# facebookresearch/seamless_communication

Measured on AMD Instinct MI355X. Metric: S2ST utterances/sec (and real-time factor), seamlessM4T_v2_large, 10 s audio, higher is better.
Workload: dtype f32 activations x f16 weights, f32 accumulate

## Files before the change

### include/seamless_hip_internal.h

```cpp
#ifndef SEAMLESS_HIP_INTERNAL_H_
#define SEAMLESS_HIP_INTERNAL_H_

#include "seamless_hip.h"

#ifdef __cplusplus
extern "C" {
#endif

int sc_decoder_step_family(sc_model* m, int rows, int caller);

int sc_op_knob(const char* name, int dflt);

int sc_op_force_general_gemm(int on);
int32_t sc_op_voc_pack_plan(const int32_t* h_need, int32_t n, int64_t budget_rows, int32_t* h_group_first, int32_t cap);
int32_t sc_op_voc_tile_first(const int32_t* h_off, int32_t n, int32_t mul, int32_t tile_rows, int32_t* h_first);
int32_t sc_op_last_vocoder_packed_groups(sc_model* m);
int sc_op_single_plane(int on);
int sc_op_layernorm(const float* d_x, const float* d_gamma, const float* d_beta, float* d_y, int32_t rows, int32_t C,
                    int32_t act);
int sc_op_linear(const float* d_x, const void* d_w_f16, const float* d_bias, const float* d_res, float* d_y,
                 int32_t M, int32_t N, int32_t K, int32_t act, float alpha, int32_t split, int32_t force_gemv);
int sc_op_skinny_linear(const float* d_x, const void* d_w_f16, const float* d_bias, const float* d_res, float* d_y,
                        int32_t M, int32_t N, int32_t K, int32_t act, float alpha);
int sc_op_skinny_res_ln(const float* d_in, const void* d_w_f16, const float* d_bias, float* d_x_inout,
// ... 42 lines not shown
int sc_op_xattn_rows(const float* d_q, int64_t ldq, const float* d_k, int64_t ldk, int32_t n, int32_t s1, int32_t s_enc, int32_t heads,
                     const int32_t* h_enc_lens, const int32_t* h_tok_lens, float* d_xattn);
int32_t sc_op_xattn_rows_tile(int32_t which);
int sc_op_conv1d_presplit(const float* d_x, const void* d_w_f16_packed, const float* d_bias, const float* d_res, float* d_y,
                          void* d_yh_f16, void* d_yl_f16, int32_t nb, int32_t t, int32_t cin, int32_t cout, int32_t k, int32_t pad,
                          int32_t dil, const unsigned char* d_row_valid, int32_t act);
int sc_op_resblock_pair_ps(const float* d_x, const void* d_w1_packed, const float* d_b1, const void* d_w2_packed, const float* d_b2,
                           float* d_out, int32_t nb, int32_t T, int32_t C, int32_t k, int32_t dil);
int sc_op_resblock_pair(const float* d_x, const void* d_w1_packed, const float* d_b1, const void* d_w2_packed,
                        const float* d_b2, float* d_out, int32_t nb, int32_t T, int32_t C, int32_t k, int32_t dil,
                        float slope, const float* d_avg_a, const float* d_avg_b);
int sc_op_mrf_fused(const float* d_x, const void* const* d_w1_packed, const float* const* d_b1, const void* const* d_w2_packed,
                    const float* const* d_b2, float* d_out, int32_t nb, int32_t T, int32_t C, const int32_t* k, const int32_t* dil,
                    float slope);
int sc_op_attention(const float* d_q, const float* d_k, const float* d_v, float* d_out, int32_t nb, int32_t heads,
                    int32_t sq, int32_t skv, int64_t ldq, int64_t ldk, int64_t ldv, int64_t ldo,
                    const int32_t* d_kv_lens, int32_t causal, const float* d_rel_k, int32_t rel_left,
                    int32_t rel_right);
int sc_op_attention_ex(const float* d_q, const float* d_k, const float* d_v, float* d_out, int32_t nb, int32_t heads,
                       int32_t sq, int32_t skv, int64_t ldq, int64_t ldk, int64_t ldv, int64_t ldo,
                       const int32_t* d_kv_lens, int32_t causal, const float* d_rel_k, int32_t rel_left,
                       int32_t rel_right, const int32_t* d_row_off, const float* d_rp_table, int64_t rp_ld,
                       const float* d_q_bias_u, const float* d_q_bias_v, void* d_out_hi, void* d_out_lo, int64_t ldoh);
int sc_op_glu_dwconv(const float* d_x, const float* d_w, float* d_y, int32_t nb, int32_t T, int32_t C, int32_t k,
                     const int32_t* d_lens);
int sc_op_glu_dwconv_ln(const float* d_x, const float* d_w, const float* d_gamma, const float* d_beta, int32_t act, void* d_yh_f16,
                        void* d_yl_f16, int32_t nb, int32_t T, int32_t C, int32_t k, const int32_t* d_lens, int32_t fused);
int sc_op_layernorm2(const float* d_x, const float* d_ga, const float* d_ba, const float* d_gb, const float* d_bb, float* d_y,
                     void* d_yh_f16, void* d_yl_f16, int32_t rows, int32_t C, int32_t fused);
int sc_op_argmax(const float* d_logits, int32_t rows, int32_t V, int32_t* d_idx, float* d_lprob);

int sc_op_beam_candidates(float* d_logits, int64_t ld, int32_t n_utt, int32_t beams, int32_t V, const float* d_cum, int32_t first_step,
                          int32_t no_eos, int32_t force_eos, int32_t pad_idx, int32_t eos_idx, int32_t unk_idx, float unk_penalty, int32_t K,
                          float* d_cand_val, int32_t* d_cand_idx, const int32_t* d_seqs, int32_t seq_ld, int32_t S, int32_t G,
                          const int32_t* d_rows, const int32_t* d_slots, int32_t chunked);
int sc_op_beam_candidates_banned(float* d_logits, int64_t ld, int32_t n_utt, int32_t beams, int32_t V, const float* d_cum,
                                 int32_t first_step, int32_t no_eos, int32_t force_eos, int32_t pad_idx, int32_t eos_idx, int32_t unk_idx,
                                 float unk_penalty, int32_t K, float* d_cand_val, int32_t* d_cand_idx, const int32_t* d_seqs,
                                 int32_t seq_ld, int32_t S, int32_t G, const int32_t* d_rows, const int32_t* d_slots, int32_t chunked,
                                 const int32_t* d_banned_tokens, const int32_t* d_banned_offsets, int32_t n_banned);
int sc_op_sample_rows(float* d_logits, int64_t ld, int32_t rows, int32_t V, const uint64_t* d_stream, const int32_t* d_gen,
                      const int32_t* d_position, float temperature, int32_t top_k, float top_p, uint64_t seed, int32_t no_eos, int32_t force_eos,
                      int32_t pad_idx, int32_t eos_idx, int32_t unk_idx, float unk_penalty, const int32_t* d_seqs, int32_t seq_ld, int32_t S,
                      int32_t G, const int32_t* d_banned_tokens, const int32_t* d_banned_offsets, int32_t n_banned, int32_t* d_tok,
                      float* d_lprob, int32_t* d_kept, uint64_t* d_z_kept);
int sc_op_beam_select(const float* d_cand_val, const int32_t* d_cand_idx, const int32_t* d_seqs_cur, int32_t* d_seqs_new, float* d_fin_score,
// ... 104 lines not shown
```

### seamless_communication_amd/_lib.py

```python
from __future__ import annotations

import ctypes as C
from pathlib import Path
from typing import Optional

import os

_VARIANT = os.environ.get("SC_LIB_VARIANT", "")
LIB_PATH = Path(__file__).resolve().parent / (f"libseamless_hip.{_VARIANT}.so" if _VARIANT else "libseamless_hip.so")

SC_ABI_VERSION = 10
SC_MAX_UPSAMPLES = 8
SC_MAX_RESBLOCK_KERNELS = 4
SC_MAX_RESBLOCK_DILATIONS = 4
SC_F16, SC_F32, SC_I32 = 0, 1, 2


class SeamlessHipError(RuntimeError):
    pass


class sc_tensor_desc(C.Structure):
    _fields_ = [
        ("name", C.c_char_p),
# ... 257 lines not shown
    "sc_op_glu_dwconv_ln": (C.c_int, [_P, _P, _P, _P, _i, _P, _P, _i, _i, _i, _i, _P, _i]),
    "sc_op_layernorm2": (C.c_int, [_P, _P, _P, _P, _P, _P, _P, _P, _i, _i, _i]),
    "sc_op_dstep3_gemv": (C.c_int, [_i, _P, _P, _P, _P, _P, _P, _P, _P, _i, _i, _i, _i, _i, _i]),
    "sc_op_dstep3_argmax": (C.c_int, [_P, _P, _i, _i, _i, _i, _i, _i, _i, _i, _i, C.c_float, _P, _P]),
    "sc_op_chain_bench": (C.c_int, [_i, _i, _i, _i, _P]),
    "sc_op_dstep_attention": (C.c_int, [_P, _i, _P, _P, _P, _i, _i, _P, _i, _i, _i, _P]),
    "sc_op_conv1d": (C.c_int, [_P, _P, _P, _P, _P, _i, _i, _i, _i, _i, _i, _i, _i, _P, _i, _i]),
    "sc_op_pack_conv_weight": (C.c_int, [_P, _P, _i, _i, _i]),
    "sc_op_conv_transpose1d": (C.c_int, [_P, _P, _P, _P, _P, _i, _i, _i, _i, _i, _i, _i, _i]),
    "sc_op_linear_presplit": (C.c_int, [_P, _P, _P, _P, _P, _P, _P, _i, _i, _i, _i, C.c_float]),
    "sc_op_linear_presplit_argmax": (C.c_int, [_P, _P, _P, _P, _i, _i, _i]),
    "sc_op_linear_presplit_score": (C.c_int, [_P, _P, _P, _P, _P, _P, _P, _P, _i, _i, _i]),
    "sc_op_linear_presplit_score_grouped": (C.c_int, [_P, _P, _P, _P, _P, _P, _P, _P, _i, _i, _i, _i]),
    "sc_op_score_candidates": (C.c_int, [_P, _P, _P, _P, _i, _P, _P, _i, _i, _i]),
    "sc_op_score_record_cols": (_i, [_i]),
    "sc_op_score_group_rows": (_i, [_i]),
    "sc_op_conv1d_presplit": (C.c_int, [_P, _P, _P, _P, _P, _P, _P, _i, _i, _i, _i, _i, _i, _i, _P, _i]),
    "sc_op_mrf_fused": (C.c_int, [_P, _P, _P, _P, _P, _P, _i, _i, _i, _P, _P, C.c_float]),
    "sc_op_resblock_pair": (C.c_int, [_P, _P, _P, _P, _P, _P, _i, _i, _i, _i, _i, C.c_float, _P, _P]),
    "sc_op_attention": (C.c_int, [_P, _P, _P, _P, _i, _i, _i, _i, C.c_int64, C.c_int64, C.c_int64, C.c_int64, _P, _i,
                                  _P, _i, _i]),
    "sc_op_attention_ex": (C.c_int, [_P, _P, _P, _P, _i, _i, _i, _i, C.c_int64, C.c_int64, C.c_int64, C.c_int64, _P, _i,
                                     _P, _i, _i, _P, _P, C.c_int64, _P, _P, _P, _P, C.c_int64]),
    "sc_op_glu_dwconv": (C.c_int, [_P, _P, _P, _i, _i, _i, _i, _P]),
    "sc_op_argmax": (C.c_int, [_P, _i, _i, _P, _P]),
    "sc_op_beam_candidates": (C.c_int, [_P, C.c_int64, _i, _i, _i, _P, _i, _i, _i, _i, _i, _i, C.c_float, _i, _P, _P, _P, _i, _i, _i,
                                        _P, _P, _i]),
    "sc_op_beam_candidates_banned": (C.c_int, [_P, C.c_int64, _i, _i, _i, _P, _i, _i, _i, _i, _i, _i, C.c_float, _i, _P, _P, _P, _i, _i,
                                               _i, _P, _P, _i, _P, _P, _i]),
    "sc_op_sample_rows": (C.c_int, [_P, C.c_int64, _i, _i, _P, _P, _P, C.c_float, _i, C.c_float, C.c_uint64, _i, _i, _i, _i, _i, C.c_float,
                                    _P, _i, _i, _i, _P, _P, _i, _P, _P, _P, _P]),
    "sc_op_beam_select": (C.c_int, [_P, _P, _P, _P, _P, _P, _P, _P, _P, _P, _P, _P, _P, _P, _i, _P, _P, _i, _i, _i, _i, _i, _i, _i, _i,
                                    _i, C.c_float]),
    "sc_op_beam_compact": (C.c_int, [_P, _P, _P, _P, _P, _P, _P, _P, _P, _i, _i, _i, _i, _i, _i]),
    "sc_op_gather_cache": (C.c_int, [_P, _P, _P, _i, _i, _i, _i, _i, C.c_int64]),
    "sc_op_row_token_lprob": (C.c_int, [_P, C.c_int64, _i, _i, _i, _i, _P]),
    "sc_op_dstep_attention_ex": (C.c_int, [_P, _i, _P, _P, _P, _i, _i, _i, _P, _i, _i, _i, _P, _P, _P, _P, _i, _P, _P]),
    "sc_op_engine_step_close": (C.c_int, [_P, _P, _i, _i, _i, _i, _i, _i, _i, C.c_float, _P, _P, _i, _i, _P, _P, _P, _P, _P, _P, _P, _P]),
    "sc_op_engine_admit": (C.c_int, [_P, _i, _i, _i, _i, _P, _P, _P, _P, _P, _P, _P, _P, _P]),
    "sc_op_engine_set_slots": (C.c_int, [_P, _i, _i, _i, _P, _P, _P, _P]),
    "sc_op_engine_retire": (C.c_int, [_P, _P, _P, _i, _i, _i, _i, _P, _P, _P, _P, _P]),
    "sc_op_dstep3_embed_ex": (C.c_int, [_P, _P, C.c_float, _P, _i, _P, _P, _i, _i, _i, _i, _i, _P]),
    "sc_op_dstep3_reduce_capture_ex": (C.c_int, [_P, _i, _P, _P, _P, _P, _P, _P, C.c_int64, _i, _i, _P, _P, _i, _i, _i]),
    "sc_op_step_update": (C.c_int, [_P, _P, _i, _P, _P, _P, _P, _i, _i, _i, _i, _P]),
    "sc_op_row_swap": (C.c_int, [_P, _P, _P, _i, _i, _P, _P, _i, _i, _i, _i, _i, _P, _P, _P, _P, _P, _P, _P, _P]),
}
# ... 92 lines not shown
```

### seamless_communication_amd/csrc/api.hip

```cpp
#include <atomic>
#include <cstring>
#include <map>
#include <mutex>
#include <set>

#include "engine.h"
#include "handle.h"

using namespace sc;

struct sc_model {
    Model m;
    sc_config& cfg = m.cfg;
};

struct sc_engine {
    std::unique_ptr<Engine> e;
    int device = 0;
    const void* weights = nullptr;
    std::set<sc_model*> attached;
};

static std::mutex g_attach_mu;
static std::map<Engine*, sc_engine*> g_engine_owner;
// ... 1453 lines not shown
    SC_CHECK(d_x && d_w1_packed && d_b1 && d_w2_packed && d_b2 && d_out && k && dil, "sc_op_mrf_fused: null argument");
    MrfArgs a;
    a.x = d_x;
    a.out = d_out;
    a.nb = nb;
    a.T = T;
    a.C = C;
    a.slope = slope;
    for (int j = 0; j < 3; ++j) a.k[j] = k[j];
    for (int q = 0; q < 9; ++q) {
        a.dil[q] = dil[q];
        a.w1[q] = static_cast<const __half*>(d_w1_packed[q]);
        a.w2[q] = static_cast<const __half*>(d_w2_packed[q]);
        a.ldw1[q] = a.ldw2[q] = align_up((int64_t)C * k[q / 3], 32);
        a.b1[q] = d_b1[q];
        a.b2[q] = d_b2[q];
    }
    a.single = g_op_single.load();
    launch_mrf_fused(a, g_op_stream);
    SC_HIP(hipStreamSynchronize(g_op_stream));
    SC_API_END
}

int sc_op_attention(const float* d_q, const float* d_k, const float* d_v, float* d_out, int32_t nb, int32_t heads,
                    int32_t sq, int32_t skv, int64_t ldq, int64_t ldk, int64_t ldv, int64_t ldo, const int32_t* d_kv_lens,
                    int32_t causal, const float* d_rel_k, int32_t rel_left, int32_t rel_right) {
    SC_API_BEGIN
    AttnArgs a;
    a.q = d_q;
    a.k = d_k;
    a.v = d_v;
    a.out = d_out;
    a.ldq = ldq;
    a.ldk = ldk;
    a.ldv = ldv;
    a.ldo = ldo;
    a.nb = nb;
    a.heads = heads;
    a.Sq = sq;
    a.Skv = skv;
    a.kv_lens = d_kv_lens;
    a.causal = causal;
    a.rel_k = d_rel_k;
    a.rel_left = rel_left;
    a.rel_right = rel_right;
    launch_attention(a, g_op_stream);
    SC_HIP(hipStreamSynchronize(g_op_stream));
    SC_API_END
}

int sc_op_attention_ex(const float* d_q, const float* d_k, const float* d_v, float* d_out, int32_t nb, int32_t heads,
                       int32_t sq, int32_t skv, int64_t ldq, int64_t ldk, int64_t ldv, int64_t ldo, const int32_t* d_kv_lens,
                       int32_t causal, const float* d_rel_k, int32_t rel_left, int32_t rel_right, const int32_t* d_row_off,
                       const float* d_rp_table, int64_t rp_ld, const float* d_q_bias_u, const float* d_q_bias_v, void* d_out_hi,
                       void* d_out_lo, int64_t ldoh) {
    SC_API_BEGIN
    AttnArgs a;
    a.q = d_q;
    a.k = d_k;
    a.v = d_v;
    a.out = d_out;
    a.ldq = ldq;
    a.ldk = ldk;
    a.ldv = ldv;
    a.ldo = ldo;
    a.nb = nb;
    a.heads = heads;
    a.Sq = sq;
    a.Skv = skv;
    a.kv_lens = d_kv_lens;
    a.causal = causal;
    a.rel_k = d_rel_k;
    a.rel_left = rel_left;
    a.rel_right = rel_right;
    a.row_off = d_row_off;
    a.rp_table = d_rp_table;
    a.rp_ld = rp_ld;
    a.q_bias_u = d_q_bias_u;
    a.q_bias_v = d_q_bias_v;
    a.out_hi = static_cast<__half*>(d_out_hi);
// ... 495 lines not shown
```

### seamless_communication_amd/csrc/k_attn.hip

```cpp
#include <cstdlib>

#include "device_util.h"

namespace sc {

static constexpr int HD = 64;

static constexpr int MQ = 128;
static constexpr int MKV = 32;
static constexpr int KS = 68;
static constexpr int KH_LD = 72;
static constexpr int VT_LD = 40;

template <int MODE>
__global__ __launch_bounds__(256) void attn_mfma16_kernel(AttnArgs p) {
    constexpr bool SHAW = MODE == 1;
    constexpr bool RELPOS = MODE == 2;
    extern __shared__ __attribute__((aligned(16))) float smem[];
    _Float16* sKh = reinterpret_cast<_Float16*>(smem);
    _Float16* sKl = sKh + MKV * KH_LD;
    _Float16* sVh = sKl + MKV * KH_LD;
    _Float16* sVl = sVh + HD * VT_LD;
    float* sQR = smem + 4 * 32 * KS;
    float* sT = smem + 4 * 32 * KS;
    float* sR = smem;

    const int tid = threadIdx.x, lane = tid & 63, wave = tid >> 6;
    const int ql = lane & 31, hh = lane >> 5;
    int qb = blockIdx.x, h = blockIdx.y, n = blockIdx.z;
    {
        const int gx = gridDim.x, bh_all = gridDim.y * gridDim.z;
        if ((bh_all & 7) == 0) {
            const int L = blockIdx.x + gx * (blockIdx.y + gridDim.y * blockIdx.z);
            const int bh = (L / (8 * gx)) * 8 + (L & 7);
            qb = (L >> 3) % gx;
            h = bh % gridDim.y;
            n = bh / gridDim.y;
        }
    }
    const int q0 = qb * MQ + wave * 32;
    const int qi = q0 + ql;
    const int kv_len = p.kv_lens ? min(p.kv_lens[n], p.Skv) : p.Skv;
    const int shift = p.Skv - p.Sq;
    const int qabs = qi + shift;
    const int npos = p.rel_left + 1 + p.rel_right;
    const int sq_n = p.row_off ? kv_len : p.Sq;
    const int64_t qbase = p.row_off ? (int64_t)p.row_off[n] : (int64_t)n * p.Sq;
    const int64_t kvbase = p.row_off ? (int64_t)p.row_off[n] : (int64_t)n * p.Skv;
    if (p.row_off && qb * MQ >= kv_len) return;
    const bool qok = qi < sq_n;
    const float* qrow = p.q + (qbase + (qok ? qi : 0)) * p.ldq + h * HD;

    if (SHAW) {
        float qreg[32];
#pragma unroll
        for (int g = 0; g < 8; ++g) {
            f32x4_t v = {0.f, 0.f, 0.f, 0.f};
            if (qok) v = *reinterpret_cast<const f32x4_t*>(qrow + 8 * g + 4 * hh);
            qreg[4 * g + 0] = v[0];
            qreg[4 * g + 1] = v[1];
            qreg[4 * g + 2] = v[2];
            qreg[4 * g + 3] = v[3];
        }
        for (int idx = tid; idx < npos * (HD / 4); idx += 256) {
            const int r = idx >> 4, c4 = idx & 15;
            *reinterpret_cast<f32x4_t*>(&sR[r * KS + c4 * 4]) = *reinterpret_cast<const f32x4_t*>(p.rel_k + r * HD + c4 * 4);
        }
        __syncthreads();
#pragma unroll 1
        for (int f = 0; f < 3; ++f) {
            if (f * 32 >= npos) break;
            float16_t qr;
#pragma unroll
            for (int r = 0; r < 16; ++r) qr[r] = 0.f;
#pragma unroll
            for (int g = 0; g < 8; ++g) {
                const f32x4_t r4 = *reinterpret_cast<const f32x4_t*>(&sR[(f * 32 + ql) * KS + 8 * g + 4 * hh]);
                qr = __builtin_amdgcn_mfma_f32_32x32x2f32(r4[0], qreg[4 * g + 0], qr, 0, 0, 0);
                qr = __builtin_amdgcn_mfma_f32_32x32x2f32(r4[1], qreg[4 * g + 1], qr, 0, 0, 0);
                qr = __builtin_amdgcn_mfma_f32_32x32x2f32(r4[2], qreg[4 * g + 2], qr, 0, 0, 0);
                qr = __builtin_amdgcn_mfma_f32_32x32x2f32(r4[3], qreg[4 * g + 3], qr, 0, 0, 0);
            }
#pragma unroll
            for (int r = 0; r < 16; ++r) {
                const int e = f * 32 + (r & 3) + 8 * (r >> 2) + 4 * hh;
                if (e < npos) sQR[(wave * 32 + ql) * npos + e] = qr[r];
            }
        }
    }

    half8_t qh[4], qlo[4], qvh[RELPOS ? 4 : 1], qvl[RELPOS ? 4 : 1];
#pragma unroll
    for (int c = 0; c < 4; ++c) {
        float x[8];
#pragma unroll
        for (int e = 0; e < 8; ++e) x[e] = 0.f;
        if (qok) {
            const f32x4_t v0 = *reinterpret_cast<const f32x4_t*>(qrow + 16 * c + 8 * hh);
            const f32x4_t v1 = *reinterpret_cast<const f32x4_t*>(qrow + 16 * c + 8 * hh + 4);
#pragma unroll
            for (int e = 0; e < 4; ++e) {
                x[e] = v0[e];
                x[4 + e] = v1[e];
            }
        }
        if (RELPOS) {
            float xu[8], xv[8];
#pragma unroll
            for (int e = 0; e < 8; ++e) {
                xu[e] = x[e] + p.q_bias_u[h * HD + 16 * c + 8 * hh + e];
                xv[e] = x[e] + p.q_bias_v[h * HD + 16 * c + 8 * hh + e];
            }
            split8(xu, qh[c], qlo[c]);
            split8(xv, qvh[c], qvl[c]);
        } else {
            split8(x, qh[c], qlo[c]);
        }
    }

    float16_t o0, o1;
#pragma unroll
    for (int r = 0; r < 16; ++r) {
        o0[r] = 0.f;
        o1[r] = 0.f;
    }
    float m_i = -1e30f, l_i = 0.f;

    int k_end = kv_len;
    if (p.causal) k_end = min(k_end, qb * MQ + MQ - 1 + shift + 1);

    const int sr0 = tid >> 4, sc4 = tid & 15;
    f32x4_t kf[2], vf[2];
    auto fetch = [&](int k0) {
#pragma unroll
        for (int u = 0; u < 2; ++u) {
            const int r = sr0 + 16 * u;
            kf[u] = f32x4_t{0.f, 0.f, 0.f, 0.f};
            vf[u] = kf[u];
            if (k0 + r < kv_len) {
                const int64_t row = kvbase + k0 + r;
                kf[u] = *reinterpret_cast<const f32x4_t*>(p.k + row * p.ldk + h * HD + sc4 * 4);
                vf[u] = *reinterpret_cast<const f32x4_t*>(p.v + row * p.ldv + h * HD + sc4 * 4);
            }
        }
    };
    if (k_end > 0) fetch(0);

    for (int k0 = 0; k0 < k_end; k0 += MKV) {
        __syncthreads();
#pragma unroll
        for (int u = 0; u < 2; ++u) {
            const int r = sr0 + 16 * u;
            half4_t khi, klo, vhi, vlo;
#pragma unroll
            for (int e = 0; e < 4; ++e) {
                const _Float16 a = (_Float16)kf[u][e];
                khi[e] = a;
                klo[e] = (_Float16)(kf[u][e] - (float)a);
                const _Float16 b = (_Float16)vf[u][e];
                vhi[e] = b;
                vlo[e] = (_Float16)(vf[u][e] - (float)b);
            }
            *reinterpret_cast<half4_t*>(&sKh[r * KH_LD + 4 * sc4]) = khi;
            *reinterpret_cast<half4_t*>(&sKl[r * KH_LD + 4 * sc4]) = klo;
            const int w = r & 15;
            const int pos = (r & 16) + 8 * ((w >> 2) & 1) + (w & 3) + 4 * (w >> 3);
#pragma unroll
            for (int e = 0; e < 4; ++e) {
                sVh[(4 * sc4 + e) * VT_LD + pos] = vhi[e];
                sVl[(4 * sc4 + e) * VT_LD + pos] = vlo[e];
            }
        }
        if (k0 + MKV < k_end) fetch(k0 + MKV);
        __syncthreads();

        float qr[16];
        if (SHAW) {
            const float* qrow_t = sQR + (wave * 32 + ql) * npos;
            const int rel_max = k0 + (MKV - 1) - (q0 + shift);
            const int rel_min = k0 - (q0 + 31 + shift);
            if (rel_max <= -p.rel_left) {
                const float v = qrow_t[0];
#pragma unroll
                for (int r = 0; r < 16; ++r) qr[r] = v;
            } else if (rel_min >= p.rel_right) {
                const float v = qrow_t[npos - 1];
#pragma unroll
                for (int r = 0; r < 16; ++r) qr[r] = v;
            } else {
#pragma unroll
                for (int r = 0; r < 16; ++r) {
                    const int kj = k0 + (r & 3) + 8 * (r >> 2) + 4 * hh;
                    const int rel = max(-p.rel_left, min(p.rel_right, kj - qabs)) + p.rel_left;
                    qr[r] = qrow_t[rel];
                }
            }
        }
        if (RELPOS) {
            const int t0w = (p.Skv - 1) - (q0 + shift) + k0 - 31;
            const int t_max = 2 * p.Skv - 2;
            float* tw = sT + wave * (64 * 32);
#pragma unroll
            for (int blk = 0; blk < 2; ++blk) {
                const int trow = min(max(t0w + blk * 32 + ql, 0), t_max);
                const float* rrow = p.rp_table + (int64_t)trow * p.rp_ld + h * HD + 8 * hh;
                f32x4_t ra[4][2];
#pragma unroll
                for (int c = 0; c < 4; ++c) {
                    ra[c][0] = *reinterpret_cast<const f32x4_t*>(rrow + 16 * c);
                    ra[c][1] = *reinterpret_cast<const f32x4_t*>(rrow + 16 * c + 4);
                }
                float16_t tt;
#pragma unroll
                for (int r = 0; r < 16; ++r) tt[r] = 0.f;
#pragma unroll
                for (int c = 0; c < 4; ++c) {
                    float x[8];
#pragma unroll
                    for (int e = 0; e < 4; ++e) {
                        x[e] = ra[c][0][e];
                        x[4 + e] = ra[c][1][e];
                    }
                    half8_t rh, rl;
                    split8(x, rh, rl);
                    tt = __builtin_amdgcn_mfma_f32_32x32x16_f16(rh, qvh[c], tt, 0, 0, 0);
                    tt = __builtin_amdgcn_mfma_f32_32x32x16_f16(rh, qvl[c], tt, 0, 0, 0);
                    tt = __builtin_amdgcn_mfma_f32_32x32x16_f16(rl, qvh[c], tt, 0, 0, 0);
                }
#pragma unroll
                for (int r = 0; r < 16; ++r) tw[(blk * 32 + (r & 3) + 8 * (r >> 2) + 4 * hh) * 32 + ql] = tt[r];
            }
#pragma unroll
            for (int r = 0; r < 16; ++r) {
                const int jl = (r & 3) + 8 * (r >> 2) + 4 * hh;
                qr[r] = tw[(jl - ql + 31) * 32 + ql];
            }
        }
        float16_t st;
#pragma unroll
        for (int r = 0; r < 16; ++r) st[r] = 0.f;
#pragma unroll
        for (int c = 0; c < 4; ++c) {
            const half8_t kh = *reinterpret_cast<const half8_t*>(&sKh[ql * KH_LD + 16 * c + 8 * hh]);
            const half8_t kl = *reinterpret_cast<const half8_t*>(&sKl[ql * KH_LD + 16 * c + 8 * hh]);
            st = __builtin_amdgcn_mfma_f32_32x32x16_f16(kh, qh[c], st, 0, 0, 0);
            st = __builtin_amdgcn_mfma_f32_32x32x16_f16(kh, qlo[c], st, 0, 0, 0);
            st = __builtin_amdgcn_mfma_f32_32x32x16_f16(kl, qh[c], st, 0, 0, 0);
        }
        float mx = -INFINITY;
#pragma unroll
        for (int r = 0; r < 16; ++r) {
            const int kj = k0 + (r & 3) + 8 * (r >> 2) + 4 * hh;
            float sc = st[r];
            if (SHAW || RELPOS) sc += qr[r];
            const bool ok = (kj < kv_len) && (!p.causal || kj <= qabs);
            sc = sc * 0.125f + (ok ? 0.f : -INFINITY);
            st[r] = sc;
            mx = fmaxf(mx, sc);
        }
        mx = fmaxf(mx, __shfl_xor(mx, 32));
        const float m_new = fmaxf(m_i, mx);
        constexpr float LOG2E = 1.44269504088896340736f;
        const float alpha = __builtin_amdgcn_exp2f((m_i - m_new) * LOG2E);
        float rs = 0.f;
#pragma unroll
        for (int r = 0; r < 16; ++r) {
            const float pv = __builtin_amdgcn_exp2f((st[r] - m_new) * LOG2E);
            st[r] = pv;
            rs += pv;
        }
        rs += __shfl_xor(rs, 32);
        l_i = l_i * alpha + rs;
        m_i = m_new;
        if (__builtin_amdgcn_ballot_w64(alpha != 1.f) != 0) {
#pragma unroll
            for (int r = 0; r < 16; ++r) {
                o0[r] *= alpha;
                o1[r] *= alpha;
            }
        }
#pragma unroll
        for (int c = 0; c < 2; ++c) {
            float x[8];
#pragma unroll
            for (int e = 0; e < 8; ++e) x[e] = st[8 * c + e];
            half8_t ph, pl;
            split8(x, ph, pl);
            const half8_t v0h = *reinterpret_cast<const half8_t*>(&sVh[ql * VT_LD + 16 * c + 8 * hh]);
            const half8_t v0l = *reinterpret_cast<const half8_t*>(&sVl[ql * VT_LD + 16 * c + 8 * hh]);
            const half8_t v1h = *reinterpret_cast<const half8_t*>(&sVh[(32 + ql) * VT_LD + 16 * c + 8 * hh]);
            const half8_t v1l = *reinterpret_cast<const half8_t*>(&sVl[(32 + ql) * VT_LD + 16 * c + 8 * hh]);
            o0 = __builtin_amdgcn_mfma_f32_32x32x16_f16(v0h, ph, o0, 0, 0, 0);
            o1 = __builtin_amdgcn_mfma_f32_32x32x16_f16(v1h, ph, o1, 0, 0, 0);
            o0 = __builtin_amdgcn_mfma_f32_32x32x16_f16(v0h, pl, o0, 0, 0, 0);
            o1 = __builtin_amdgcn_mfma_f32_32x32x16_f16(v1h, pl, o1, 0, 0, 0);
            o0 = __builtin_amdgcn_mfma_f32_32x32x16_f16(v0l, ph, o0, 0, 0, 0);
            o1 = __builtin_amdgcn_mfma_f32_32x32x16_f16(v1l, ph, o1, 0, 0, 0);
        }
    }

    __syncthreads();
    float* ot = smem + wave * (32 * KS);
    const float inv = l_i > 0.f ? 1.0f / l_i : 0.f;
#pragma unroll
    for (int r = 0; r < 16; ++r) {
        const int d = (r & 3) + 8 * (r >> 2) + 4 * hh;
        ot[ql * KS + d] = o0[r] * inv;
        ot[ql * KS + 32 + d] = o1[r] * inv;
    }
#pragma unroll
    for (int it = 0; it < 8; ++it) {
        const int row = it * 4 + (lane >> 4);
        const int c0 = (lane & 15) * 4;
        const int qq = q0 + row;
        const f32x4_t of = *reinterpret_cast<const f32x4_t*>(&ot[row * KS + c0]);
        if (qq >= sq_n) continue;
        if (p.out_hi) {
            const half4_t hi = __builtin_convertvector(of, half4_t);
            const f32x4_t back = __builtin_convertvector(hi, f32x4_t);
            const int64_t off = (qbase + qq) * p.ldoh + h * HD + c0;
            *reinterpret_cast<half4_t*>(p.out_hi + off) = hi;
            *reinterpret_cast<half4_t*>(p.out_lo + off) = __builtin_convertvector(of - back, half4_t);
        } else {
            *reinterpret_cast<f32x4_t*>(p.out + (qbase + qq) * p.ldo + h * HD + c0) = of;
        }
    }
}

static bool g_attn_attr_set = false;

void launch_attention(const AttnArgs& a, hipStream_t s) {
    if (a.head_dim == 80 || a.head_dim == 128) {
        launch_attention_hd(a, s);
        return;
    }
    SC_CHECK(a.head_dim == HD, "attention: head_dim=%d (64, 80 and 128 exist)", a.head_dim);
    SC_CHECK(a.nb > 0 && a.heads > 0 && a.Sq > 0 && a.Skv > 0, "attention: empty problem");
    SC_CHECK(a.out || (a.out_hi && a.out_lo && a.ldoh % 4 == 0), "attention: no output");
    SC_CHECK(a.ldq % 4 == 0 && a.ldk % 4 == 0 && a.ldv % 4 == 0 && a.ldo % 4 == 0 && (reinterpret_cast<uintptr_t>(a.out) & 15) == 0,
             "attention: row strides must be multiples of 4 and the output 16-byte aligned");
    const int npos = a.rel_left + 1 + a.rel_right;
    SC_CHECK(npos <= 96, "attention: %d relative positions > 96", npos);
    SC_CHECK(!a.row_off || (a.kv_lens && a.Sq == a.Skv && !a.causal), "attention: packed rows need kv_lens and Sq == Skv");
    if (a.rp_table)
        SC_CHECK(!a.rel_k && !a.causal && a.Sq == a.Skv && a.q_bias_u && a.q_bias_v && a.rp_ld % 4 == 0,
                 "attention: relative positions need self-attention (Sq == Skv), both query biases and a 16-byte aligned table");
    if (!g_attn_attr_set) {
        SC_HIP(hipFuncSetAttribute(reinterpret_cast<const void*>(&attn_mfma16_kernel<0>), hipFuncAttributeMaxDynamicSharedMemorySize, 120 * 1024));
        SC_HIP(hipFuncSetAttribute(reinterpret_cast<const void*>(&attn_mfma16_kernel<1>), hipFuncAttributeMaxDynamicSharedMemorySize, 120 * 1024));
        SC_HIP(hipFuncSetAttribute(reinterpret_cast<const void*>(&attn_mfma16_kernel<2>), hipFuncAttributeMaxDynamicSharedMemorySize, 120 * 1024));
        g_attn_attr_set = true;
    }
    const double pairs = a.pairs > 0 ? a.pairs : (double)a.nb * a.Sq * a.Skv;
    prof::Scope scope(a.rel_k ? "attention_shaw" : "attention", 4.0 * a.heads * pairs * HD,
                      4.0 * a.nb * a.heads * HD * (2.0 * a.Sq + 2.0 * a.Skv), s);
    size_t lds = (size_t)(4 * 32 * KS) * sizeof(float);
    if (a.rel_k) lds += (size_t)(MQ * npos) * sizeof(float);
    if (a.rp_table) lds += (size_t)(4 * 64 * 32) * sizeof(float);
    dim3 grid(cdiv(a.Sq, MQ), a.heads, a.nb);
    if (a.rp_table) hipLaunchKernelGGL((attn_mfma16_kernel<2>), grid, dim3(256), lds, s, a);
    else if (a.rel_k) hipLaunchKernelGGL((attn_mfma16_kernel<1>), grid, dim3(256), lds, s, a);
    else hipLaunchKernelGGL((attn_mfma16_kernel<0>), grid, dim3(256), lds, s, a);
    SC_LAUNCH_CHECK();
}

static constexpr int MAX_CACHE = 4096;

__global__ __launch_bounds__(256) void decode_attn_kernel(
    const float* __restrict__ q, int64_t ldq, const float* __restrict__ k_new,
    const float* __restrict__ v_new, int64_t ldkv, float* __restrict__ kcache,
    float* __restrict__ vcache, int64_t cache_ld, int64_t cache_bs, int cap, float* __restrict__ out,
    int64_t ldo, int heads, const int* __restrict__ d_pos, const int* __restrict__ kv_lens, int use_lens,
    int in_splits, int64_t in_split_stride, const float* __restrict__ bias_q,
    const float* __restrict__ bias_k, const float* __restrict__ bias_v) {
    __shared__ float s_q[HD];
    __shared__ float s_sc[MAX_CACHE];
    __shared__ float s_red[8];
    __shared__ float s_part[4][HD];

    const int tid = threadIdx.x, lane = tid & 63, wave = tid >> 6;
    const int h = blockIdx.x, b = blockIdx.y;
    const int pos = d_pos ? *d_pos : 0;
    const int kv_len = use_lens ? min(kv_lens[b], cap) : pos + 1;
    float* kc = kcache + (int64_t)b * cache_bs + h * HD;
    float* vc = vcache + (int64_t)b * cache_bs + h * HD;
// ... 78 lines not shown
```

### seamless_communication_amd/csrc/kernels.h

```cpp
#pragma once
#include <atomic>

#include "common.h"
#include "prof.h"

namespace sc {

enum Act { ACT_NONE = 0, ACT_RELU = 1, ACT_SILU = 2, ACT_TANH = 3, ACT_GELU = 4 };
enum InAct { IN_NONE = 0, IN_LRELU_01 = 1, IN_LRELU_001 = 2 };

__device__ __forceinline__ int argmax_stored_index(int idx) { return idx == 0x7fffffff ? 0 : idx; }

__device__ __forceinline__ float lrelu_in(float x, float slope) {
    const float r = fmaxf(x, 0.f) + slope * fminf(x, 0.f);
    return x != x ? x : r;
}

struct GemmArgs {
    const float* A = nullptr;
    int64_t lda = 0;
    const __half* W = nullptr;
    int64_t ldw = 0;
    int64_t w_phase_stride = 0;
    const float* bias = nullptr;
// ... 384 lines not shown
void launch_relpos_table(int S, int M, float* out, hipStream_t s);

struct AttnArgs {
    const float* q = nullptr;
    const float* k = nullptr;
    const float* v = nullptr;
    float* out = nullptr;
    int64_t ldq = 0, ldk = 0, ldv = 0, ldo = 0;
    int nb = 0, heads = 0, Sq = 0, Skv = 0;
    const int* kv_lens = nullptr;
    int causal = 0;
    const float* rel_k = nullptr;
    int rel_left = 0, rel_right = 0;
    const float* rp_table = nullptr;
    int64_t rp_ld = 0;
    const float* q_bias_u = nullptr;
    const float* q_bias_v = nullptr;
    const int* row_off = nullptr;
    double pairs = 0;
    __half* out_hi = nullptr;
    __half* out_lo = nullptr;
    int64_t ldoh = 0;
    int head_dim = 64;
};
void launch_attention(const AttnArgs& a, hipStream_t s);
void launch_attention_hd(const AttnArgs& a, hipStream_t s);

void launch_decode_attention(const float* q, int64_t ldq, const float* k_new, const float* v_new,
                             int64_t ldkv, float* kcache, float* vcache, int64_t cache_ld, int64_t cache_bs,
                             int cap, float* out, int64_t ldo, int nb, int heads, const int* d_pos,
                             const int* kv_lens, int use_lens, hipStream_t s, int in_splits = 1,
                             int64_t in_split_stride = 0, const float* bias_q = nullptr,
                             const float* bias_k = nullptr, const float* bias_v = nullptr);

constexpr int BANNED_MAX_SEQS = 4096, BANNED_MAX_LEN = 64, BANNED_MAX_TOKENS = 65536;
struct BannedList {
    const int* tokens = nullptr;
    const int* offsets = nullptr;
    int n = 0;
    int max_len = 0;
};
void validate_banned_host(const int32_t* tokens, const int32_t* offsets, int n_banned, int V, int* out_max_len);
void launch_beam_candidates(float* logits, int64_t ld, int n_utt, int beams, int V, const float* cum, int first_step,
                            int no_eos, int force_eos, int pad_idx, int eos_idx, int unk_idx, float unk_penalty, int K,
                            float* cand_val, int* cand_idx, const int* seqs, int seq_ld, int S, int G, hipStream_t s,
                            const int* d_slots = nullptr, const BannedList* banned = nullptr);
// ... 393 lines not shown
```

Measured before the change: 338.4.

## Add 8-wave double-buffered attention kernel variant for Shaw relative-position attention

Templates the MFMA attention kernel on wave count, adding an 8-wave (512-thread, 256-query) variant that double-buffers K/V tiles in LDS. This removes one barrier per KV tile and overlaps staging with compute. It is chosen automatically for Shaw relative-key attention without row offsets, when the query-block count is even and the LDS fits; otherwise the 4-wave path is used. It also adds a waves-per-EU hint, an API override for the wave count, and LDS sizing per variant. The cost is more LDS and registers per block, which may lower occupancy.

```diff
diff --git a/include/seamless_hip_internal.h b/include/seamless_hip_internal.h
--- a/include/seamless_hip_internal.h
+++ b/include/seamless_hip_internal.h
@@ -88,6 +88,7 @@
                        const int32_t* d_kv_lens, int32_t causal, const float* d_rel_k, int32_t rel_left,
                        int32_t rel_right, const int32_t* d_row_off, const float* d_rp_table, int64_t rp_ld,
                        const float* d_q_bias_u, const float* d_q_bias_v, void* d_out_hi, void* d_out_lo, int64_t ldoh);
+int sc_op_attention_waves(int32_t waves);
 int sc_op_glu_dwconv(const float* d_x, const float* d_w, float* d_y, int32_t nb, int32_t T, int32_t C, int32_t k,
                      const int32_t* d_lens);
 int sc_op_glu_dwconv_ln(const float* d_x, const float* d_w, const float* d_gamma, const float* d_beta, int32_t act, void* d_yh_f16,
diff --git a/seamless_communication_amd/_lib.py b/seamless_communication_amd/_lib.py
--- a/seamless_communication_amd/_lib.py
+++ b/seamless_communication_amd/_lib.py
@@ -303,6 +303,7 @@
                                   _P, _i, _i]),
     "sc_op_attention_ex": (C.c_int, [_P, _P, _P, _P, _i, _i, _i, _i, C.c_int64, C.c_int64, C.c_int64, C.c_int64, _P, _i,
                                      _P, _i, _i, _P, _P, C.c_int64, _P, _P, _P, _P, C.c_int64]),
+    "sc_op_attention_waves": (C.c_int, [_i]),
     "sc_op_glu_dwconv": (C.c_int, [_P, _P, _P, _i, _i, _i, _i, _P]),
     "sc_op_argmax": (C.c_int, [_P, _i, _i, _P, _P]),
     "sc_op_beam_candidates": (C.c_int, [_P, C.c_int64, _i, _i, _i, _P, _i, _i, _i, _i, _i, _i, C.c_float, _i, _P, _P, _P, _i, _i, _i,
diff --git a/seamless_communication_amd/csrc/api.hip b/seamless_communication_amd/csrc/api.hip
--- a/seamless_communication_amd/csrc/api.hip
+++ b/seamless_communication_amd/csrc/api.hip
@@ -1499,11 +1499,20 @@
     SC_API_END
 }
 
+static std::atomic<int> g_op_attn_waves{0};
+int sc_op_attention_waves(int32_t waves) {
+    SC_API_BEGIN
+    SC_CHECK(waves == 0 || waves == 4 || waves == 8, "sc_op_attention_waves: %d (0, 4 or 8)", waves);
+    g_op_attn_waves.store(waves);
+    SC_API_END
+}
+
 int sc_op_attention(const float* d_q, const float* d_k, const float* d_v, float* d_out, int32_t nb, int32_t heads,
                     int32_t sq, int32_t skv, int64_t ldq, int64_t ldk, int64_t ldv, int64_t ldo, const int32_t* d_kv_lens,
                     int32_t causal, const float* d_rel_k, int32_t rel_left, int32_t rel_right) {
     SC_API_BEGIN
     AttnArgs a;
+    a.force_waves = g_op_attn_waves.load();
     a.q = d_q;
     a.k = d_k;
     a.v = d_v;
@@ -1533,6 +1542,7 @@
                        void* d_out_lo, int64_t ldoh) {
     SC_API_BEGIN
     AttnArgs a;
+    a.force_waves = g_op_attn_waves.load();
     a.q = d_q;
     a.k = d_k;
     a.v = d_v;
diff --git a/seamless_communication_amd/csrc/k_attn.hip b/seamless_communication_amd/csrc/k_attn.hip
--- a/seamless_communication_amd/csrc/k_attn.hip
+++ b/seamless_communication_amd/csrc/k_attn.hip
@@ -6,23 +6,36 @@
 
 static constexpr int HD = 64;
 
-static constexpr int MQ = 128;
 static constexpr int MKV = 32;
 static constexpr int KS = 68;
 static constexpr int KH_LD = 72;
 static constexpr int VT_LD = 40;
-
-template <int MODE>
-__global__ __launch_bounds__(256) void attn_mfma16_kernel(AttnArgs p) {
+static constexpr int KV_SET = 2 * MKV * KH_LD + 2 * HD * VT_LD;
+static constexpr size_t ATTN_LDS_MAX = 160 * 1024;
+
+static constexpr int attn_region0(int nw) { return nw * 32 * KS; }
+
+static size_t attn_lds_bytes(int nw, bool shaw, bool relpos, int npos) {
+    size_t fl = attn_region0(nw);
+    if (shaw) fl += (size_t)nw * 32 * npos;
+    if (relpos) fl += (size_t)nw * 64 * 32;
+    return fl * sizeof(float);
+}
+
+template <int MODE, int NW>
+__device__ __forceinline__ void attn_mfma16_body(const AttnArgs& p) {
     constexpr bool SHAW = MODE == 1;
     constexpr bool RELPOS = MODE == 2;
+    constexpr bool DB = NW == 8;
+    constexpr int MQ = NW * 32;
+    constexpr int NT = NW * 64;
+    constexpr int NU = 512 / NT;
+    static_assert(NW == 4 || NW == 8, "4 or 8 waves");
+    static_assert(96 * KS <= attn_region0(NW) && (DB ? 2 : 1) * KV_SET <= 2 * attn_region0(NW), "what region 0 has to hold");
     extern __shared__ __attribute__((aligned(16))) float smem[];
-    _Float16* sKh = reinterpret_cast<_Float16*>(smem);
-    _Float16* sKl = sKh + MKV * KH_LD;
-    _Float16* sVh = sKl + MKV * KH_LD;
-    _Float16* sVl = sVh + HD * VT_LD;
-    float* sQR = smem + 4 * 32 * KS;
-    float* sT = smem + 4 * 32 * KS;
+    _Float16* sKV = reinterpret_cast<_Float16*>(smem);
+    float* sQR = smem + attn_region0(NW);
+    float* sT = smem + attn_region0(NW);
     float* sR = smem;
 
     const int tid = threadIdx.x, lane = tid & 63, wave = tid >> 6;
@@ -62,7 +75,7 @@
             qreg[4 * g + 2] = v[2];
             qreg[4 * g + 3] = v[3];
         }
-        for (int idx = tid; idx < npos * (HD / 4); idx += 256) {
+        for (int idx = tid; idx < npos * (HD / 4); idx += NT) {
             const int r = idx >> 4, c4 = idx & 15;
             *reinterpret_cast<f32x4_t*>(&sR[r * KS + c4 * 4]) = *reinterpret_cast<const f32x4_t*>(p.rel_k + r * HD + c4 * 4);
         }
@@ -87,6 +100,7 @@
                 if (e < npos) sQR[(wave * 32 + ql) * npos + e] = qr[r];
             }
         }
+        if (DB) __syncthreads();
     }
 
     half8_t qh[4], qlo[4], qvh[RELPOS ? 4 : 1], qvl[RELPOS ? 4 : 1];
@@ -130,11 +144,11 @@
     if (p.causal) k_end = min(k_end, qb * MQ + MQ - 1 + shift + 1);
 
     const int sr0 = tid >> 4, sc4 = tid & 15;
-    f32x4_t kf[2], vf[2];
+    f32x4_t kf[NU], vf[NU];
     auto fetch = [&](int k0) {
 #pragma unroll
-        for (int u = 0; u < 2; ++u) {
-            const int r = sr0 + 16 * u;
+        for (int u = 0; u < NU; ++u) {
+            const int r = sr0 + (NT / 16) * u;
             kf[u] = f32x4_t{0.f, 0.f, 0.f, 0.f};
             vf[u] = kf[u];
             if (k0 + r < kv_len) {
@@ -144,13 +158,14 @@
             }
         }
     };
-    if (k_end > 0) fetch(0);
-
-    for (int k0 = 0; k0 < k_end; k0 += MKV) {
-        __syncthreads();
-#pragma unroll
-        for (int u = 0; u < 2; ++u) {
-            const int r = sr0 + 16 * u;
+    auto stage = [&](int buf) {
+        _Float16* sKh = sKV + buf * KV_SET;
+        _Float16* sKl = sKh + MKV * KH_LD;
+        _Float16* sVh = sKl + MKV * KH_LD;
+        _Float16* sVl = sVh + HD * VT_LD;
+#pragma unroll
+        for (int u = 0; u < NU; ++u) {
+            const int r = sr0 + (NT / 16) * u;
             half4_t khi, klo, vhi, vlo;
 #pragma unroll
             for (int e = 0; e < 4; ++e) {
@@ -171,132 +186,158 @@
                 sVl[(4 * sc4 + e) * VT_LD + pos] = vlo[e];
             }
         }
-        if (k0 + MKV < k_end) fetch(k0 + MKV);
-        __syncthreads();
-
-        float qr[16];
-        if (SHAW) {
-            const float* qrow_t = sQR + (wave * 32 + ql) * npos;
-            const int rel_max = k0 + (MKV - 1) - (q0 + shift);
-            const int rel_min = k0 - (q0 + 31 + shift);
-            if (rel_max <= -p.rel_left) {
-                const float v = qrow_t[0];
-#pragma unroll
-                for (int r = 0; r < 16; ++r) qr[r] = v;
-            } else if (rel_min >= p.rel_right) {
-                const float v = qrow_t[npos - 1];
-#pragma unroll
-                for (int r = 0; r < 16; ++r) qr[r] = v;
-            } else {
+    };
+    if (k_end > 0) {
+        fetch(0);
+        if (DB) {
+            stage(0);
+            if (MKV < k_end) fetch(MKV);
+        }
+    }
+    const bool wave_live = __builtin_amdgcn_readfirstlane(q0) < sq_n;
+    if (DB) __syncthreads();
+
+    for (int k0 = 0; k0 < k_end; k0 += MKV) {
+        const int buf = DB ? (k0 / MKV) & 1 : 0;
+        if (!DB) {
+            __syncthreads();
+            stage(0);
+            if (k0 + MKV < k_end) fetch(k0 + MKV);
+            __syncthreads();
+        } else if (k0 + MKV < k_end) {
+            stage(buf ^ 1);
+            if (k0 + 2 * MKV < k_end) fetch(k0 + 2 * MKV);
+        }
+        if (wave_live) {
+            const _Float16* sKh = sKV + buf * KV_SET;
+            const _Float16* sKl = sKh + MKV * KH_LD;
+            const _Float16* sVh = sKl + MKV * KH_LD;
+            const _Float16* sVl = sVh + HD * VT_LD;
+            float qr[16];
+            if (SHAW) {
+                const float* qrow_t = sQR + (wave * 32 + ql) * npos;
+                const int rel_max = k0 + (MKV - 1) - (q0 + shift);
+                const int rel_min = k0 - (q0 + 31 + shift);
+                if (rel_max <= -p.rel_left) {
+                    const float v = qrow_t[0];
+#pragma unroll
+                    for (int r = 0; r < 16; ++r) qr[r] = v;
+                } else if (rel_min >= p.rel_right) {
+                    const float v = qrow_t[npos - 1];
+#pragma unroll
+                    for (int r = 0; r < 16; ++r) qr[r] = v;
+                } else {
+#pragma unroll
+                    for (int r = 0; r < 16; ++r) {
+                        const int kj = k0 + (r & 3) + 8 * (r >> 2) + 4 * hh;
+                        const int rel = max(-p.rel_left, min(p.rel_right, kj - qabs)) + p.rel_left;
+                        qr[r] = qrow_t[rel];
+                    }
+                }
+            }
+            if (RELPOS) {
+                const int t0w = (p.Skv - 1) - (q0 + shift) + k0 - 31;
+                const int t_max = 2 * p.Skv - 2;
+                float* tw = sT + wave * (64 * 32);
+#pragma unroll
+                for (int blk = 0; blk < 2; ++blk) {
+                    const int trow = min(max(t0w + blk * 32 + ql, 0), t_max);
+                    const float* rrow = p.rp_table + (int64_t)trow * p.rp_ld + h * HD + 8 * hh;
+                    f32x4_t ra[4][2];
+#pragma unroll
+                    for (int c = 0; c < 4; ++c) {
+                        ra[c][0] = *reinterpret_cast<const f32x4_t*>(rrow + 16 * c);
+                        ra[c][1] = *reinterpret_cast<const f32x4_t*>(rrow + 16 * c + 4);
+                    }
+                    float16_t tt;
+#pragma unroll
+                    for (int r = 0; r < 16; ++r) tt[r] = 0.f;
+#pragma unroll
+                    for (int c = 0; c < 4; ++c) {
+                        float x[8];
+#pragma unroll
+                        for (int e = 0; e < 4; ++e) {
+                            x[e] = ra[c][0][e];
+                            x[4 + e] = ra[c][1][e];
+                        }
+                        half8_t rh, rl;
+                        split8(x, rh, rl);
+                        tt = __builtin_amdgcn_mfma_f32_32x32x16_f16(rh, qvh[c], tt, 0, 0, 0);
+                        tt = __builtin_amdgcn_mfma_f32_32x32x16_f16(rh, qvl[c], tt, 0, 0, 0);
+                        tt = __builtin_amdgcn_mfma_f32_32x32x16_f16(rl, qvh[c], tt, 0, 0, 0);
+                    }
+#pragma unroll
+                    for (int r = 0; r < 16; ++r) tw[(blk * 32 + (r & 3) + 8 * (r >> 2) + 4 * hh) * 32 + ql] = tt[r];
+                }
 #pragma unroll
                 for (int r = 0; r < 16; ++r) {
-                    const int kj = k0 + (r & 3) + 8 * (r >> 2) + 4 * hh;
-                    const int rel = max(-p.rel_left, min(p.rel_right, kj - qabs)) + p.rel_left;
-                    qr[r] = qrow_t[rel];
+                    const int jl = (r & 3) + 8 * (r >> 2) + 4 * hh;
+                    qr[r] = tw[(jl - ql + 31) * 32 + ql];
                 }
             }
-        }
-        if (RELPOS) {
-            const int t0w = (p.Skv - 1) - (q0 + shift) + k0 - 31;
-            const int t_max = 2 * p.Skv - 2;
-            float* tw = sT + wave * (64 * 32);
-#pragma unroll
-            for (int blk = 0; blk < 2; ++blk) {
-                const int trow = min(max(t0w + blk * 32 + ql, 0), t_max);
-                const float* rrow = p.rp_table + (int64_t)trow * p.rp_ld + h * HD + 8 * hh;
-                f32x4_t ra[4][2];
-#pragma unroll
-                for (int c = 0; c < 4; ++c) {
-                    ra[c][0] = *reinterpret_cast<const f32x4_t*>(rrow + 16 * c);
-                    ra[c][1] = *reinterpret_cast<const f32x4_t*>(rrow + 16 * c + 4);
+            float16_t st;
+#pragma unroll
+            for (int r = 0; r < 16; ++r) st[r] = 0.f;
+#pragma unroll
+            for (int c = 0; c < 4; ++c) {
+                const half8_t kh = *reinterpret_cast<const half8_t*>(&sKh[ql * KH_LD + 16 * c + 8 * hh]);
+                const half8_t kl = *reinterpret_cast<const half8_t*>(&sKl[ql * KH_LD + 16 * c + 8 * hh]);
+                st = __builtin_amdgcn_mfma_f32_32x32x16_f16(kh, qh[c], st, 0, 0, 0);
+                st = __builtin_amdgcn_mfma_f32_32x32x16_f16(kh, qlo[c], st, 0, 0, 0);
+                st = __builtin_amdgcn_mfma_f32_32x32x16_f16(kl, qh[c], st, 0, 0, 0);
+            }
+            float mx = -INFINITY;
+#pragma unroll
+            for (int r = 0; r < 16; ++r) {
+                const int kj = k0 + (r & 3) + 8 * (r >> 2) + 4 * hh;
+                float sc = st[r];
+                if (SHAW || RELPOS) sc += qr[r];
+                const bool ok = (kj < kv_len) && (!p.causal || kj <= qabs);
+                sc = sc * 0.125f + (ok ? 0.f : -INFINITY);
+                st[r] = sc;
+                mx = fmaxf(mx, sc);
+            }
+            mx = fmaxf(mx, __shfl_xor(mx, 32));
+            const float m_new = fmaxf(m_i, mx);
+            constexpr float LOG2E = 1.44269504088896340736f;
+            const float alpha = __builtin_amdgcn_exp2f((m_i - m_new) * LOG2E);
+            float rs = 0.f;
+#pragma unroll
+            for (int r = 0; r < 16; ++r) {
+                const float pv = __builtin_amdgcn_exp2f((st[r] - m_new) * LOG2E);
+                st[r] = pv;
+                rs += pv;
+            }
+            rs += __shfl_xor(rs, 32);
+            l_i = l_i * alpha + rs;
+            m_i = m_new;
+            if (__builtin_amdgcn_ballot_w64(alpha != 1.f) != 0) {
+#pragma unroll
+                for (int r = 0; r < 16; ++r) {
+                    o0[r] *= alpha;
+                    o1[r] *= alpha;
                 }
-                float16_t tt;
-#pragma unroll
-                for (int r = 0; r < 16; ++r) tt[r] = 0.f;
-#pragma unroll
-                for (int c = 0; c < 4; ++c) {
-                    float x[8];
-#pragma unroll
-                    for (int e = 0; e < 4; ++e) {
-                        x[e] = ra[c][0][e];
-                        x[4 + e] = ra[c][1][e];
-                    }
-                    half8_t rh, rl;
-                    split8(x, rh, rl);
-                    tt = __builtin_amdgcn_mfma_f32_32x32x16_f16(rh, qvh[c], tt, 0, 0, 0);
-                    tt = __builtin_amdgcn_mfma_f32_32x32x16_f16(rh, qvl[c], tt, 0, 0, 0);
-                    tt = __builtin_amdgcn_mfma_f32_32x32x16_f16(rl, qvh[c], tt, 0, 0, 0);
-                }
-#pragma unroll
-                for (int r = 0; r < 16; ++r) tw[(blk * 32 + (r & 3) + 8 * (r >> 2) + 4 * hh) * 32 + ql] = tt[r];
-            }
-#pragma unroll
-            for (int r = 0; r < 16; ++r) {
-                const int jl = (r & 3) + 8 * (r >> 2) + 4 * hh;
-                qr[r] = tw[(jl - ql + 31) * 32 + ql];
-            }
-        }
-        float16_t st;
-#pragma unroll
-        for (int r = 0; r < 16; ++r) st[r] = 0.f;
-#pragma unroll
-        for (int c = 0; c < 4; ++c) {
-            const half8_t kh = *reinterpret_cast<const half8_t*>(&sKh[ql * KH_LD + 16 * c + 8 * hh]);
-            const half8_t kl = *reinterpret_cast<const half8_t*>(&sKl[ql * KH_LD + 16 * c + 8 * hh]);
-            st = __builtin_amdgcn_mfma_f32_32x32x16_f16(kh, qh[c], st, 0, 0, 0);
-            st = __builtin_amdgcn_mfma_f32_32x32x16_f16(kh, qlo[c], st, 0, 0, 0);
-            st = __builtin_amdgcn_mfma_f32_32x32x16_f16(kl, qh[c], st, 0, 0, 0);
-        }
-        float mx = -INFINITY;
-#pragma unroll
-        for (int r = 0; r < 16; ++r) {
-            const int kj = k0 + (r & 3) + 8 * (r >> 2) + 4 * hh;
-            float sc = st[r];
-            if (SHAW || RELPOS) sc += qr[r];
-            const bool ok = (kj < kv_len) && (!p.causal || kj <= qabs);
-            sc = sc * 0.125f + (ok ? 0.f : -INFINITY);
-            st[r] = sc;
-            mx = fmaxf(mx, sc);
-        }
-        mx = fmaxf(mx, __shfl_xor(mx, 32));
-        const float m_new = fmaxf(m_i, mx);
-        constexpr float LOG2E = 1.44269504088896340736f;
-        const float alpha = __builtin_amdgcn_exp2f((m_i - m_new) * LOG2E);
-        float rs = 0.f;
-#pragma unroll
-        for (int r = 0; r < 16; ++r) {
-            const float pv = __builtin_amdgcn_exp2f((st[r] - m_new) * LOG2E);
-            st[r] = pv;
-            rs += pv;
-        }
-        rs += __shfl_xor(rs, 32);
-        l_i = l_i * alpha + rs;
-        m_i = m_new;
-        if (__builtin_amdgcn_ballot_w64(alpha != 1.f) != 0) {
-#pragma unroll
-            for (int r = 0; r < 16; ++r) {
-                o0[r] *= alpha;
-                o1[r] *= alpha;
-            }
-        }
-#pragma unroll
-        for (int c = 0; c < 2; ++c) {
-            float x[8];
-#pragma unroll
-            for (int e = 0; e < 8; ++e) x[e] = st[8 * c + e];
-            half8_t ph, pl;
-            split8(x, ph, pl);
-            const half8_t v0h = *reinterpret_cast<const half8_t*>(&sVh[ql * VT_LD + 16 * c + 8 * hh]);
-            const half8_t v0l = *reinterpret_cast<const half8_t*>(&sVl[ql * VT_LD + 16 * c + 8 * hh]);
-            const half8_t v1h = *reinterpret_cast<const half8_t*>(&sVh[(32 + ql) * VT_LD + 16 * c + 8 * hh]);
-            const half8_t v1l = *reinterpret_cast<const half8_t*>(&sVl[(32 + ql) * VT_LD + 16 * c + 8 * hh]);
-            o0 = __builtin_amdgcn_mfma_f32_32x32x16_f16(v0h, ph, o0, 0, 0, 0);
-            o1 = __builtin_amdgcn_mfma_f32_32x32x16_f16(v1h, ph, o1, 0, 0, 0);
-            o0 = __builtin_amdgcn_mfma_f32_32x32x16_f16(v0h, pl, o0, 0, 0, 0);
-            o1 = __builtin_amdgcn_mfma_f32_32x32x16_f16(v1h, pl, o1, 0, 0, 0);
-            o0 = __builtin_amdgcn_mfma_f32_32x32x16_f16(v0l, ph, o0, 0, 0, 0);
-            o1 = __builtin_amdgcn_mfma_f32_32x32x16_f16(v1l, ph, o1, 0, 0, 0);
-        }
+            }
+#pragma unroll
+            for (int c = 0; c < 2; ++c) {
+                float x[8];
+#pragma unroll
+                for (int e = 0; e < 8; ++e) x[e] = st[8 * c + e];
+                half8_t ph, pl;
+                split8(x, ph, pl);
+                const half8_t v0h = *reinterpret_cast<const half8_t*>(&sVh[ql * VT_LD + 16 * c + 8 * hh]);
+                const half8_t v0l = *reinterpret_cast<const half8_t*>(&sVl[ql * VT_LD + 16 * c + 8 * hh]);
+                const half8_t v1h = *reinterpret_cast<const half8_t*>(&sVh[(32 + ql) * VT_LD + 16 * c + 8 * hh]);
+                const half8_t v1l = *reinterpret_cast<const half8_t*>(&sVl[(32 + ql) * VT_LD + 16 * c + 8 * hh]);
+                o0 = __builtin_amdgcn_mfma_f32_32x32x16_f16(v0h, ph, o0, 0, 0, 0);
+                o1 = __builtin_amdgcn_mfma_f32_32x32x16_f16(v1h, ph, o1, 0, 0, 0);
+                o0 = __builtin_amdgcn_mfma_f32_32x32x16_f16(v0h, pl, o0, 0, 0, 0);
+                o1 = __builtin_amdgcn_mfma_f32_32x32x16_f16(v1h, pl, o1, 0, 0, 0);
+                o0 = __builtin_amdgcn_mfma_f32_32x32x16_f16(v0l, ph, o0, 0, 0, 0);
+                o1 = __builtin_amdgcn_mfma_f32_32x32x16_f16(v1l, ph, o1, 0, 0, 0);
+            }
+        }
+        if (DB && k0 + MKV < k_end) __syncthreads();
     }
 
     __syncthreads();
@@ -327,7 +368,41 @@
     }
 }
 
+template <int MODE>
+__global__ __launch_bounds__(256) __attribute__((amdgpu_waves_per_eu(2))) void attn_mfma16_kernel(AttnArgs p) {
+    attn_mfma16_body<MODE, 4>(p);
+}
+template <int MODE>
+__global__ __launch_bounds__(512) __attribute__((amdgpu_waves_per_eu(2))) void attn_mfma16_w8_kernel(AttnArgs p) {
+    attn_mfma16_body<MODE, 8>(p);
+}
+
 static bool g_attn_attr_set = false;
+
+template <int MODE>
+static void attn_set_lds() {
+    const size_t l4 = attn_lds_bytes(4, MODE == 1, MODE == 2, 96), l8 = attn_lds_bytes(8, MODE == 1, MODE == 2, 96);
+    SC_HIP(hipFuncSetAttribute(reinterpret_cast<const void*>(&attn_mfma16_kernel<MODE>), hipFuncAttributeMaxDynamicSharedMemorySize,
+                               (int)(l4 < ATTN_LDS_MAX ? l4 : ATTN_LDS_MAX)));
+    SC_HIP(hipFuncSetAttribute(reinterpret_cast<const void*>(&attn_mfma16_w8_kernel<MODE>), hipFuncAttributeMaxDynamicSharedMemorySize,
+                               (int)(l8 < ATTN_LDS_MAX ? l8 : ATTN_LDS_MAX)));
+}
+
+template <int MODE>
+static void attn_launch(const AttnArgs& a, int nw, size_t lds, hipStream_t s) {
+    const dim3 grid(cdiv(a.Sq, nw * 32), a.heads, a.nb);
+    if (nw == 8) hipLaunchKernelGGL((attn_mfma16_w8_kernel<MODE>), grid, dim3(512), lds, s, a);
+    else hipLaunchKernelGGL((attn_mfma16_kernel<MODE>), grid, dim3(256), lds, s, a);
+}
+
+static int attn_waves(const AttnArgs& a, int npos) {
+    if (a.force_waves) {
+        SC_CHECK(a.force_waves == 4 || a.force_waves == 8, "attention: force_waves=%d (0, 4 or 8)", a.force_waves);
+        return a.force_waves;
+    }
+    const bool pairs_up = cdiv(a.Sq, 128) % 2 == 0;
+    return a.rel_k && !a.row_off && pairs_up && attn_lds_bytes(8, true, false, npos) <= ATTN_LDS_MAX ? 8 : 4;
+}
 
 void launch_attention(const AttnArgs& a, hipStream_t s) {
     if (a.head_dim == 80 || a.head_dim == 128) {
@@ -346,21 +421,20 @@
         SC_CHECK(!a.rel_k && !a.causal && a.Sq == a.Skv && a.q_bias_u && a.q_bias_v && a.rp_ld % 4 == 0,
                  "attention: relative positions need self-attention (Sq == Skv), both query biases and a 16-byte aligned table");
     if (!g_attn_attr_set) {
-        SC_HIP(hipFuncSetAttribute(reinterpret_cast<const void*>(&attn_mfma16_kernel<0>), hipFuncAttributeMaxDynamicSharedMemorySize, 120 * 1024));
-        SC_HIP(hipFuncSetAttribute(reinterpret_cast<const void*>(&attn_mfma16_kernel<1>), hipFuncAttributeMaxDynamicSharedMemorySize, 120 * 1024));
-        SC_HIP(hipFuncSetAttribute(reinterpret_cast<const void*>(&attn_mfma16_kernel<2>), hipFuncAttributeMaxDynamicSharedMemorySize, 120 * 1024));
+        attn_set_lds<0>();
+        attn_set_lds<1>();
+        attn_set_lds<2>();
         g_attn_attr_set = true;
     }
     const double pairs = a.pairs > 0 ? a.pairs : (double)a.nb * a.Sq * a.Skv;
     prof::Scope scope(a.rel_k ? "attention_shaw" : "attention", 4.0 * a.heads * pairs * HD,
                       4.0 * a.nb * a.heads * HD * (2.0 * a.Sq + 2.0 * a.Skv), s);
-    size_t lds = (size_t)(4 * 32 * KS) * sizeof(float);
-    if (a.rel_k) lds += (size_t)(MQ * npos) * sizeof(float);
-    if (a.rp_table) lds += (size_t)(4 * 64 * 32) * sizeof(float);
-    dim3 grid(cdiv(a.Sq, MQ), a.heads, a.nb);
-    if (a.rp_table) hipLaunchKernelGGL((attn_mfma16_kernel<2>), grid, dim3(256), lds, s, a);
-    else if (a.rel_k) hipLaunchKernelGGL((attn_mfma16_kernel<1>), grid, dim3(256), lds, s, a);
-    else hipLaunchKernelGGL((attn_mfma16_kernel<0>), grid, dim3(256), lds, s, a);
+    const int nw = attn_waves(a, npos);
+    const size_t lds = attn_lds_bytes(nw, a.rel_k != nullptr, a.rp_table != nullptr, npos);
+    SC_CHECK(lds <= ATTN_LDS_MAX, "attention: %d waves need %zu B of LDS > %zu", nw, lds, ATTN_LDS_MAX);
+    if (a.rp_table) attn_launch<2>(a, nw, lds, s);
+    else if (a.rel_k) attn_launch<1>(a, nw, lds, s);
+    else attn_launch<0>(a, nw, lds, s);
     SC_LAUNCH_CHECK();
 }
 
diff --git a/seamless_communication_amd/csrc/kernels.h b/seamless_communication_amd/csrc/kernels.h
--- a/seamless_communication_amd/csrc/kernels.h
+++ b/seamless_communication_amd/csrc/kernels.h
@@ -430,6 +430,7 @@
     __half* out_lo = nullptr;
     int64_t ldoh = 0;
     int head_dim = 64;
+    int force_waves = 0;
 };
 void launch_attention(const AttnArgs& a, hipStream_t s);
 void launch_attention_hd(const AttnArgs& a, hipStream_t s);
```

New measurement: 338.8, median of 6. About the same (+0.1%).
